# williamyang1991/VToonify

Hardware: NVIDIA H100
Metric: frames/sec at 576x1024 (higher is better)
Workload: dtype bf16x3 (fp32 operands split into bf16 hi+lo, 3 tensor-core products, fp32 accumulate)

## Files before the change

vtoonify_b200/csrc/conv_tc.cu:

```cuda
#include "tc_common.cuh"
#include <cuda_bf16.h>
#include <mutex>

using namespace vt_tc;

int vt_validate_conv_desc(const vt_conv_desc* d, const char* who);
extern int g_upfirdn_tiled;
extern int g_smalln_is;
extern int g_fir4;
extern int g_instnorm_chunks;
extern int g_rs_kernel;
int vt_conv_rs_takes(const vt_conv_desc* d);
int vt_conv_rs_run(const vt_conv_desc* d, void* stream);

namespace {

constexpr int TILE_W = 8, TILE_H = 16, TILE_M = 128;
constexpr int KCH = 32;
constexpr int MAX_SMEM = 227 * 1024;
constexpr int MAX_BLOCK_N = 128;
constexpr int MAX_ACC_COLS = 128;
constexpr int WIDE_N = 256;
constexpr int WIDE_REGS_XFORM = 88;
constexpr int WIDE_REGS_CONSUMER = 208;
constexpr int STATS_WARPS = 8;

struct TcArgs {
  CUtensorMap in_map[2][4];
  CUtensorMap w_map;
  int n_src, kchunks[2], coff[2];
  int n_steps;
  int8_t step_view[VT_MAX_TAPS], step_vx[VT_MAX_TAPS], step_vy[VT_MAX_TAPS];
  int16_t step_w[VT_MAX_TAPS];
  int step_aoff[VT_MAX_TAPS];
  int n_phase;
  int tgroup;
  int halo, halo_x0, halo_y0, halo_w;
  int n_hv, hv_view[4], hv_x0[4], hv_y0[4], hv_off[4], hv_bytes[4], a_rows;
  uint16_t step_sbo[VT_MAX_TAPS];
  int a_stages, b_stages, a_stage_bytes, b_stage_bytes, a_tx_bytes, b_tx_bytes;
  int block_n, n_tiles, tiles_x, tiles_y, B, total_tiles;
  int m_first;
  int Ho, Wo, Cout, wB, out_cpitch;
  const float* bias;
  const float* noise;
  const float* noise_w;
  const float* res;
  float* out;
  int64_t out_sb, out_sy, out_sx, phase_off[4];
  int64_t pix_sb, pix_sy, pix_sx, phase_pix[4];
  int act, round_tf32;
  float slope, gain, alpha, beta;
  const float* rgb_w; const float* rgb_bias; const float* rgb_skip; const float* rgb_skip_kernel; float* rgb_out;
  const float* slope_vec;
  const float* src_scale[2];
  const float* src_affine[2];
  int src_cn[2];
  int64_t sc_sb, sc_sy, sc_sx;
  int in_w, in_h;
  int mma_n;
  int m_major;
  float* stats_ws;
  float acc_scale;
};

constexpr int TC_THREADS = 384;
constexpr int XFORM_WARPS = 3;
constexpr int CONSUMERS = 2;
constexpr int RELEASE_ARRIVALS = CONSUMERS * 4;

enum TcOp : int {
  OP_TF32 = 0,
  OP_BF16 = 1,
  OP_F16 = 2,
  OP_BF16_NSTACK = 3,
};

template <int NW, bool F16>
__device__ __forceinline__ void wgmma_split(float* acc, uint64_t a, uint64_t b, uint32_t accumulate) {
  if constexpr (NW == 32) {
    if constexpr (F16) wgmma_f16_n32(acc, a, b, accumulate); else wgmma_bf16_n32(acc, a, b, accumulate);
  } else if constexpr (NW == 64) {
    if constexpr (F16) wgmma_f16_n64(acc, a, b, accumulate); else wgmma_bf16_n64(acc, a, b, accumulate);
  } else if constexpr (NW == 128) {
    if constexpr (F16) wgmma_f16_n128(acc, a, b, accumulate); else wgmma_bf16_n128(acc, a, b, accumulate);
  } else {
    static_assert(NW == WIDE_N && !F16, "the 256-wide MMA exists for the bf16 split only");
    wgmma_bf16_n256(acc, a, b, accumulate);
  }
}

template <int NW, int OP>
__device__ __forceinline__ void mma_step(float* acc, uint64_t adesc, uint64_t bdesc, uint32_t first) {
  if constexpr (OP == OP_TF32) {
    if constexpr (NW == 32) {
      wgmma_tf32_n32(acc, adesc, bdesc, first ^ 1u); wgmma_tf32_n32(acc, adesc + 2, bdesc + 2, 1);
      wgmma_tf32_n32(acc, adesc + 4, bdesc + 4, 1); wgmma_tf32_n32(acc, adesc + 6, bdesc + 6, 1);
    } else if constexpr (NW == 64) {
      wgmma_tf32_n64(acc, adesc, bdesc, first ^ 1u); wgmma_tf32_n64(acc, adesc + 2, bdesc + 2, 1);
      wgmma_tf32_n64(acc, adesc + 4, bdesc + 4, 1); wgmma_tf32_n64(acc, adesc + 6, bdesc + 6, 1);
    } else {
      wgmma_tf32_n128(acc, adesc, bdesc, first ^ 1u); wgmma_tf32_n128(acc, adesc + 2, bdesc + 2, 1);
      wgmma_tf32_n128(acc, adesc + 4, bdesc + 4, 1); wgmma_tf32_n128(acc, adesc + 6, bdesc + 6, 1);
    }
  } else {
    constexpr bool nstack = OP == OP_BF16_NSTACK;
    constexpr int ao[6] = {0, 2, 4, 6, 0, 2};
    constexpr int bo[6] = {0, 2, 0, 2, 4, 6};
#pragma unroll
    for (int i = 0; i < (nstack ? 4 : 6); ++i)
      wgmma_split<NW, OP == OP_F16>(acc, adesc + (uint64_t)ao[i], bdesc + (uint64_t)(nstack ? ao[i] : bo[i]), i == 0 ? (first ^ 1u) : 1u);
  }
}

template <int NW, int MT, int OP>
__global__ void __launch_bounds__(TC_THREADS, 1)
conv_tc_kernel(const __grid_constant__ TcArgs p) {
  constexpr bool WIDE = NW == WIDE_N;
  static_assert((MT * NW <= MAX_ACC_COLS || (WIDE && MT == 1 && OP == OP_BF16)) && (MT == 1 || MT == 2 || MT == 4),
                "accumulators of one work item exceed the register plan");
  static_assert(128 * WIDE_REGS_XFORM + 256 * WIDE_REGS_CONSUMER <= TC_THREADS * ((65536 / TC_THREADS) & ~7),
                "setmaxnreg plan exceeds the launch allocation");
  static_assert(OP != OP_BF16_NSTACK || NW == 64, "the N-stacked form is the Cout == 32 layer at MMA N = 64");
  constexpr bool SPLIT = OP != OP_TF32;
  extern __shared__ uint8_t smem_raw[];
  const uint32_t smem_base = (smem_u32(smem_raw) + 1023u) & ~1023u;
  const uint32_t a_base = smem_base;
  const uint32_t b_base = a_base + (uint32_t)p.a_stages * p.a_stage_bytes;
  const uint32_t bar_base = b_base + (uint32_t)p.b_stages * p.b_stage_bytes;
  auto a_full = [&](int i) { return bar_base + 8u * i; };
  auto a_empty = [&](int i) { return bar_base + 64u + 8u * i; };
  auto b_full = [&](int i) { return bar_base + 128u + 8u * i; };
  auto b_empty = [&](int i) { return bar_base + 192u + 8u * i; };
  auto a_ready = [&](int i) { return bar_base + 256u + 8u * i; };

  const int warp = threadIdx.x >> 5, lane = threadIdx.x & 31;
  const int wg = threadIdx.x >> 7;

  if (warp == 0 && lane == 0) {
    for (int s = 0; s < p.n_src; ++s)
      for (int v = 0; v < 4; ++v) tma_prefetch_desc(&p.in_map[s][v]);
    tma_prefetch_desc(&p.w_map);
  }
  if (warp == 1 && lane == 0) {
    for (int i = 0; i < p.a_stages; ++i) { mbar_init(a_full(i), 1); mbar_init(a_empty(i), RELEASE_ARRIVALS); mbar_init(a_ready(i), XFORM_WARPS); }
    for (int i = 0; i < p.b_stages; ++i) { mbar_init(b_full(i), 1); mbar_init(b_empty(i), RELEASE_ARRIVALS); }
    fence_barrier_init();
    fence_proxy_async_smem();
  }
  __syncthreads();

  const int m_tiles = p.total_tiles / p.n_tiles;
  const int tiles_per_img = p.tiles_y * p.tiles_x;
  constexpr int item_w = TILE_W * MT;

  if (wg == 0) {
    if constexpr (WIDE) asm volatile("setmaxnreg.dec.sync.aligned.u32 %0;" ::"n"(WIDE_REGS_XFORM));
    if (warp == 0) {
      int a_st = 0, b_st = 0;
      uint32_t a_par = 0, b_par = 0;
      for (int tile = blockIdx.x; tile < p.total_tiles; tile += gridDim.x) {
        const int n_tile = p.m_major ? tile % p.n_tiles : tile / m_tiles, m = p.m_first + (p.m_major ? tile / p.n_tiles : tile % m_tiles);
        const int b = m / tiles_per_img, rem = m % tiles_per_img;
        const int oy0 = (rem / p.tiles_x) * TILE_H, ox0 = (rem % p.tiles_x) * item_w;
        const int n0 = n_tile * p.block_n;
        const int wb = p.wB > 1 ? b : 0;
        for (int s = 0; s < p.n_src; ++s) {
          for (int kc = 0; kc < p.kchunks[s]; ++kc) {
            const int c0 = kc * KCH;
            if (p.halo) {
              mbar_wait(a_empty(a_st), a_par ^ 1);
              if (elect_one()) {
                const uint32_t st = a_base + a_st * p.a_stage_bytes;
                mbar_arrive_expect_tx(a_full(a_st), (uint32_t)p.a_tx_bytes);
                for (int v = 0; v < p.n_hv; ++v)
                  tma_load_4d(st + p.hv_off[v], &p.in_map[s][p.hv_view[v]], a_full(a_st), c0, ox0 + p.hv_x0[v], oy0 + p.hv_y0[v], b);
              }
              __syncwarp();
              if (++a_st == p.a_stages) { a_st = 0; a_par ^= 1; }
            }
            int gj = 0;
            for (int j = 0; j < p.n_steps; ++j) {
              if (!p.halo) {
                mbar_wait(a_empty(a_st), a_par ^ 1);
                if (elect_one()) {
                  mbar_arrive_expect_tx(a_full(a_st), (uint32_t)p.a_tx_bytes);
                  tma_load_4d(a_base + a_st * p.a_stage_bytes, &p.in_map[s][p.step_view[j]], a_full(a_st), c0, ox0 + p.step_vx[j],
                              oy0 + p.step_vy[j], b);
                }
                __syncwarp();
                if (++a_st == p.a_stages) { a_st = 0; a_par ^= 1; }
              }
              if (gj == 0) {
                mbar_wait(b_empty(b_st), b_par ^ 1);
                if (elect_one()) {
                  const int wc = SPLIT ? (p.coff[s] + c0) * 2 : p.coff[s] + c0;
                  mbar_arrive_expect_tx(b_full(b_st), (uint32_t)p.b_tx_bytes);
                  tma_load_4d(b_base + b_st * p.b_stage_bytes, &p.w_map, b_full(b_st), wc, OP == OP_BF16_NSTACK ? 0 : n0, p.step_w[j], wb);
                }
                __syncwarp();
                if (++b_st == p.b_stages) { b_st = 0; b_par ^= 1; }
              }
              if (++gj == p.tgroup) gj = 0;
            }
          }
        }
      }
    } else if constexpr (SPLIT) {
      const int t = (warp - 1) * 32 + lane;
      const int rows = p.a_rows;
      int a_st = 0;
      uint32_t a_par = 0;
      const int bw = p.halo ? p.halo_w : TILE_W;
      for (int tile = blockIdx.x; tile < p.total_tiles; tile += gridDim.x) {
        const int m = p.m_first + (p.m_major ? tile / p.n_tiles : tile % m_tiles);
        const int b = m / tiles_per_img, rem = m % tiles_per_img;
        const int oy0 = (rem / p.tiles_x) * TILE_H, ox0 = (rem % p.tiles_x) * item_w;
        for (int s = 0; s < p.n_src; ++s) {
          const float* sc = p.src_scale[s];
          const float* aff = p.src_affine[s];
          for (int kc = 0; kc < p.kchunks[s]; ++kc) {
            const float4* affp = aff ? reinterpret_cast<const float4*>(aff + ((int64_t)b * p.src_cn[s] + kc * KCH) * 2) : nullptr;
            const int loads = p.halo ? 1 : p.n_steps;
            for (int l = 0; l < loads; ++l) {
              mbar_wait(a_full(a_st), a_par);
              const uint32_t stage = a_base + a_st * p.a_stage_bytes;
              const int bx0 = ox0 + (p.halo ? p.halo_x0 : p.step_vx[l]), by0 = oy0 + (p.halo ? p.halo_y0 : p.step_vy[l]);
              for (int r = t; r < rows; r += 32 * XFORM_WARPS) {
                const uint32_t row = stage + (uint32_t)r * 128u;
                const uint32_t ph = (row >> 7) & 7u;
                float f[32];
#pragma unroll
                for (int j = 0; j < 8; ++j) {
                  float4 v;
                  asm volatile("ld.shared.v4.f32 {%0, %1, %2, %3}, [%4];" : "=f"(v.x), "=f"(v.y), "=f"(v.z), "=f"(v.w) : "r"(row + ((j ^ ph) << 4)));
                  f[4 * j] = v.x; f[4 * j + 1] = v.y; f[4 * j + 2] = v.z; f[4 * j + 3] = v.w;
                }
                if (sc || aff) {
                  const int ry = r / bw, rx = r - ry * bw;
                  const int ix = bx0 + rx, iy = by0 + ry;
                  const bool inb = ix >= 0 && ix < p.in_w && iy >= 0 && iy < p.in_h;
                  if (aff && inb) {
#pragma unroll
                    for (int j = 0; j < 16; ++j) {
                      const float4 q = __ldg(affp + j);
                      f[2 * j] = fmaf(f[2 * j], q.x, q.y);
                      f[2 * j + 1] = fmaf(f[2 * j + 1], q.z, q.w);
                    }
                  }
                  if (sc) {
                    const float mm = inb ? __ldg(sc + (int64_t)b * p.sc_sb + (int64_t)iy * p.sc_sy + (int64_t)ix * p.sc_sx) : 0.f;
#pragma unroll
                    for (int i = 0; i < 32; ++i) f[i] *= mm;
                  }
                }
                uint32_t hi[16], lo[16];
                if constexpr (OP == OP_F16) {
#pragma unroll
                  for (int i = 0; i < 16; ++i) split_f16x2(f[2 * i], f[2 * i + 1], hi[i], lo[i]);
                } else {
#pragma unroll
                  for (int i = 0; i < 16; ++i) {
                    const __nv_bfloat162 h2 = __floats2bfloat162_rn(f[2 * i], f[2 * i + 1]);
                    hi[i] = *reinterpret_cast<const uint32_t*>(&h2);
                    const float r0 = f[2 * i] - __uint_as_float(hi[i] << 16), r1 = f[2 * i + 1] - __uint_as_float(hi[i] & 0xffff0000u);
                    const __nv_bfloat162 l2 = __floats2bfloat162_rn(r0, r1);
                    lo[i] = *reinterpret_cast<const uint32_t*>(&l2);
                  }
                }
#pragma unroll
                for (int m4 = 0; m4 < 4; ++m4) {
                  asm volatile("st.shared.v4.b32 [%0], {%1, %2, %3, %4};" ::"r"(row + ((m4 ^ ph) << 4)), "r"(hi[4 * m4]), "r"(hi[4 * m4 + 1]), "r"(hi[4 * m4 + 2]), "r"(hi[4 * m4 + 3]) : "memory");
                  asm volatile("st.shared.v4.b32 [%0], {%1, %2, %3, %4};" ::"r"(row + (((m4 + 4) ^ ph) << 4)), "r"(lo[4 * m4]), "r"(lo[4 * m4 + 1]), "r"(lo[4 * m4 + 2]), "r"(lo[4 * m4 + 3]) : "memory");
                }
              }
              fence_proxy_async_smem();
              __syncwarp();
              if (lane == 0) mbar_arrive(a_ready(a_st));
              if (++a_st == p.a_stages) { a_st = 0; a_par ^= 1; }
            }
          }
        }
      }
    }
  } else {
    if constexpr (WIDE) asm volatile("setmaxnreg.inc.sync.aligned.u32 %0;" ::"n"(WIDE_REGS_CONSUMER));
    const int c = wg - 1;
    const int tw_ = (threadIdx.x & 127) >> 5;
    const bool leader = lane == 0;
    const int qd = lane & 3;
    float acc[MT][NW / 2];
#pragma unroll
    for (int g = 0; g < MT; ++g)
#pragma unroll
      for (int i = 0; i < NW / 2; ++i) acc[g][i] = 0.f;
    const float nw = (p.noise && p.noise_w) ? *p.noise_w : 0.f;
    int a_st = 0, b_st = 0;
    uint32_t a_par = 0, b_par = 0;
    const uint32_t tile_bytes_n = (uint32_t)p.mma_n * 128u;
    for (int tile = blockIdx.x; tile < p.total_tiles; tile += gridDim.x) {
      const int n_tile = p.m_major ? tile % p.n_tiles : tile / m_tiles, m = p.m_first + (p.m_major ? tile / p.n_tiles : tile % m_tiles);
      const int b = m / tiles_per_img, rem = m % tiles_per_img;
      const int oy0 = (rem / p.tiles_x) * TILE_H, ox0 = (rem % p.tiles_x) * item_w;
      const int n0 = n_tile * p.block_n;
      uint32_t first = 1;
      int rel_a = -1, rel_b = -1;
      for (int s = 0; s < p.n_src; ++s) {
        for (int kc = 0; kc < p.kchunks[s]; ++kc) {
          if (p.halo) mbar_wait(SPLIT ? a_ready(a_st) : a_full(a_st), a_par);
          int gj = 0;
          for (int j = 0; j < p.n_steps; ++j) {
            if (!p.halo) mbar_wait(SPLIT ? a_ready(a_st) : a_full(a_st), a_par);
            if (gj == 0) mbar_wait(b_full(b_st), b_par);
            uint32_t a_addr = a_base + a_st * p.a_stage_bytes;
            uint32_t sbo = 1024;
            if (p.halo) {
              a_addr += (uint32_t)p.step_aoff[j];
              sbo = (uint32_t)p.step_sbo[j];
            }
            a_addr += 8u * (uint32_t)c * sbo;
            const uint64_t bdesc = make_smem_desc_sw128(b_base + b_st * p.b_stage_bytes + (uint32_t)gj * tile_bytes_n, 1024);
            const bool last_of_group = (gj == p.tgroup - 1);
            wgmma_fence();
#pragma unroll
            for (int g = 0; g < MT; ++g) {
              const uint64_t adesc = make_smem_desc_sw128(a_addr + (uint32_t)(g * TILE_W * 128), sbo);
              mma_step<NW, OP>(acc[g], adesc, bdesc, first);
            }
            wgmma_commit();
            wgmma_wait<1>();
            if (leader) {
              if (rel_a >= 0) mbar_arrive(a_empty(rel_a));
              if (rel_b >= 0) mbar_arrive(b_empty(rel_b));
            }
            rel_a = (!p.halo || j == p.n_steps - 1) ? a_st : -1;
            rel_b = last_of_group ? b_st : -1;
            first = 0;
            if (last_of_group) { gj = 0; if (++b_st == p.b_stages) { b_st = 0; b_par ^= 1; } } else { ++gj; }
            if (!p.halo || j == p.n_steps - 1) { if (++a_st == p.a_stages) { a_st = 0; a_par ^= 1; } }
          }
        }
      }
      wgmma_wait<0>();
#pragma unroll
      for (int g = 0; g < MT; ++g) wgmma_pin<NW / 2>(acc[g]);
      if (leader) {
        if (rel_a >= 0) mbar_arrive(a_empty(rel_a));
        if (rel_b >= 0) mbar_arrive(b_empty(rel_b));
      }

      const int r0 = 64 * c + 16 * tw_ + (lane >> 2);
      const int ty = r0 / TILE_W, tx = r0 % TILE_W;
      const int ph0 = n0 / p.Cout, nb0 = n0 - ph0 * p.Cout;
      const int nchunks = p.block_n / 32;
#pragma unroll
      for (int g = 0; g < MT; ++g) {
        int oy[2], ox[2];
        bool in_img[2];
        int64_t off0[2], pix0[2];
        float rgb[2][3] = {{0.f, 0.f, 0.f}, {0.f, 0.f, 0.f}};
#pragma unroll
        for (int h = 0; h < 2; ++h) {
          oy[h] = oy0 + ty + h; ox[h] = ox0 + g * TILE_W + tx;
          in_img[h] = oy[h] < p.Ho && ox[h] < p.Wo;
          off0[h] = (int64_t)b * p.out_sb + (int64_t)oy[h] * p.out_sy + (int64_t)ox[h] * p.out_sx;
          pix0[h] = (int64_t)b * p.pix_sb + (int64_t)oy[h] * p.pix_sy + (int64_t)ox[h] * p.pix_sx;
        }
        int ph = ph0, nb = nb0 - 32;
#pragma unroll
        for (int j = 0; j < NW / 32; ++j) {
          if (j >= nchunks) break;
          nb += 32;
          if (nb >= p.Cout) { nb -= p.Cout; ++ph; }
          float nz[2];
#pragma unroll
          for (int h = 0; h < 2; ++h) nz[h] = (p.noise && in_img[h]) ? nw * __ldg(p.noise + p.phase_pix[ph] + pix0[h]) : 0.f;
          float v[2][4][2];
#pragma unroll
          for (int k = 0; k < 4; ++k)
#pragma unroll
            for (int h = 0; h < 2; ++h)
#pragma unroll
              for (int e = 0; e < 2; ++e) {
                const int i = 16 * j + 4 * k + 2 * h + e;
                float x = acc[g][i];
                if constexpr (OP == OP_BF16_NSTACK) x += acc[g][(i + 16) % (NW / 2)];
                v[h][k][e] = x * p.acc_scale;
              }
#pragma unroll
          for (int k = 0; k < 4; ++k) {
            const int ch = nb + 8 * k + 2 * qd;
            float2 bq = make_float2(0.f, 0.f), sq = make_float2(p.slope, p.slope);
            if (p.bias) bq = __ldg(reinterpret_cast<const float2*>(p.bias + ch));
            if (p.slope_vec) sq = __ldg(reinterpret_cast<const float2*>(p.slope_vec + ch));
#pragma unroll
            for (int h = 0; h < 2; ++h) {
              float v0 = v[h][k][0] + bq.x + nz[h], v1 = v[h][k][1] + bq.y + nz[h];
              if (p.act == VT_ACT_LRELU) {
                v0 = vt_lrelu(v0, sq.x) * p.gain; v1 = vt_lrelu(v1, sq.y) * p.gain;
              } else if (!WIDE && p.act == VT_ACT_RELU_TANH) {
                v0 = tanhf(fmaxf(v0, 0.f)); v1 = tanhf(fmaxf(v1, 0.f));
              }
              const int64_t off = p.phase_off[ph] + off0[h] + ch;
              if (p.res) {
                if (in_img[h]) {
                  const float2 rv = __ldg(reinterpret_cast<const float2*>(p.res + off));
                  v0 = v0 * p.alpha + p.beta * rv.x; v1 = v1 * p.alpha + p.beta * rv.y;
                }
              } else if (p.alpha != 1.f) {
                v0 *= p.alpha; v1 *= p.alpha;
              }
              if (p.round_tf32) { v0 = vt_round_tf32(v0); v1 = vt_round_tf32(v1); }
              if (!WIDE && p.rgb_w) {
                const float* w0 = p.rgb_w + ((int64_t)(p.wB > 1 ? b : 0) * 3) * p.Cout + ch;
#pragma unroll
                for (int cc = 0; cc < 3; ++cc) {
                  const float2 wv = __ldg(reinterpret_cast<const float2*>(w0 + cc * p.Cout));
                  rgb[h][cc] = fmaf(v1, wv.y, fmaf(v0, wv.x, rgb[h][cc]));
                }
              }
              if (in_img[h] && p.out) *reinterpret_cast<float2*>(p.out + off) = make_float2(v0, v1);
              v[h][k][0] = in_img[h] ? v0 : 0.f; v[h][k][1] = in_img[h] ? v1 : 0.f;
            }
          }
          if (p.stats_ws) {
            const int kchunk = ((rem * MT + g) * STATS_WARPS) + c * 4 + tw_;
            float2* wsp = reinterpret_cast<float2*>(p.stats_ws) + ((int64_t)kchunk * p.B + b) * p.Cout + nb + 2 * qd;
#pragma unroll
            for (int k = 0; k < 4; ++k)
#pragma unroll
              for (int e = 0; e < 2; ++e) {
                float ssum = v[0][k][e] + v[1][k][e];
                float ssq = fmaf(v[0][k][e], v[0][k][e], v[1][k][e] * v[1][k][e]);
#pragma unroll
                for (int o = 4; o < 32; o <<= 1) {
                  ssum += __shfl_xor_sync(0xffffffffu, ssum, o);
                  ssq += __shfl_xor_sync(0xffffffffu, ssq, o);
                }
                if (lane < 4) wsp[8 * k + e] = make_float2(ssum, ssq);
              }
          }
        }
        if (!WIDE && p.rgb_w) {
#pragma unroll
          for (int h = 0; h < 2; ++h)
#pragma unroll
            for (int cc = 0; cc < 3; ++cc) {
              rgb[h][cc] += __shfl_xor_sync(0xffffffffu, rgb[h][cc], 1);
              rgb[h][cc] += __shfl_xor_sync(0xffffffffu, rgb[h][cc], 2);
            }
#pragma unroll
          for (int h = 0; h < 2; ++h) {
            if (qd != 0 || !in_img[h]) continue;
            torgb_store(p.rgb_bias, p.rgb_skip, p.rgb_skip_kernel, p.rgb_out, rgb[h], b, oy[h], ox[h], p.Ho, p.Wo);
          }
        }
      }
    }
  }
}

struct TcKernel {
  int nw, mt, op;
  void (*fn)(TcArgs);
};
#define VT_TC_OPS(NW, MT) {NW, MT, OP_TF32, conv_tc_kernel<NW, MT, OP_TF32>}, {NW, MT, OP_BF16, conv_tc_kernel<NW, MT, OP_BF16>}, \
                          {NW, MT, OP_F16, conv_tc_kernel<NW, MT, OP_F16>}
const TcKernel kTcKernels[] = {
    VT_TC_OPS(128, 1), VT_TC_OPS(64, 1), VT_TC_OPS(64, 2), VT_TC_OPS(32, 1), VT_TC_OPS(32, 2), VT_TC_OPS(32, 4),
    {64, 1, OP_BF16_NSTACK, conv_tc_kernel<64, 1, OP_BF16_NSTACK>}, {64, 2, OP_BF16_NSTACK, conv_tc_kernel<64, 2, OP_BF16_NSTACK>},
    {WIDE_N, 1, OP_BF16, conv_tc_kernel<WIDE_N, 1, OP_BF16>},
};
#undef VT_TC_OPS

}

typedef CUresult (*PFN_encodeTiled)(CUtensorMap*, CUtensorMapDataType, cuuint32_t, void*, const cuuint64_t*,
                                    const cuuint64_t*, const cuuint32_t*, const cuuint32_t*, CUtensorMapInterleave,
                                    CUtensorMapSwizzle, CUtensorMapL2promotion, CUtensorMapFloatOOBfill);

static PFN_encodeTiled get_encode() {
  static PFN_encodeTiled fn = nullptr;
  static std::once_flag once;
  std::call_once(once, [] {
    void* f = nullptr;
    cudaDriverEntryPointQueryResult qres;
    if (cudaGetDriverEntryPoint("cuTensorMapEncodeTiled", &f, cudaEnableDefault, &qres) == cudaSuccess &&
        qres == cudaDriverEntryPointSuccess)
      fn = (PFN_encodeTiled)f;
  });
  return fn;
}

int vt_tc_make_map4(CUtensorMap* m, const void* base, const uint64_t dims[4], const uint64_t strides_b[3], const uint32_t box[4],
                    const char* what, bool bf16) {
  PFN_encodeTiled enc = get_encode();
  VT_CHECK(enc != nullptr, "conv_tc: cuTensorMapEncodeTiled not available from the driver");
  cuuint64_t gd[4] = {dims[0], dims[1], dims[2], dims[3]};
  cuuint64_t gs[3] = {strides_b[0], strides_b[1], strides_b[2]};
  cuuint32_t bx[4] = {box[0], box[1], box[2], box[3]};
  cuuint32_t es[4] = {1, 1, 1, 1};
  for (int i = 0; i < 4; ++i) VT_CHECK(gd[i] >= 1 && bx[i] >= 1 && bx[i] <= 256, "conv_tc: bad %s map dim %d (dim=%llu box=%u)", what, i, (unsigned long long)gd[i], bx[i]);
  for (int i = 0; i < 3; ++i) VT_CHECK(gs[i] % 16 == 0 && gs[i] > 0, "conv_tc: %s map stride %d (%llu B) not a positive multiple of 16", what, i, (unsigned long long)gs[i]);
  VT_CHECK(((uintptr_t)base & 15) == 0, "conv_tc: %s base pointer not 16-byte aligned", what);
  CUresult r = enc(m, bf16 ? CU_TENSOR_MAP_DATA_TYPE_BFLOAT16 : CU_TENSOR_MAP_DATA_TYPE_FLOAT32, 4, const_cast<void*>(base), gd, gs, bx, es,
                   CU_TENSOR_MAP_INTERLEAVE_NONE, CU_TENSOR_MAP_SWIZZLE_128B, CU_TENSOR_MAP_L2_PROMOTION_L2_256B,
                   CU_TENSOR_MAP_FLOAT_OOB_FILL_NONE);
  VT_CHECK(r == CUDA_SUCCESS, "conv_tc: cuTensorMapEncodeTiled(%s) failed with CUresult %d", what, (int)r);
  return 0;
}


namespace {
inline int make_map4(CUtensorMap* m, const void* base, const uint64_t dims[4], const uint64_t strides_b[3], const uint32_t box[4],
                     const char* what, bool bf16 = false) { return vt_tc_make_map4(m, base, dims, strides_b, box, what, bf16); }

int g_tc_mode = 1;
int g_tc_mt = 0;
int g_tc_transpose = 1;
int g_tc_tgroup = 0;
int g_tc_s2_halo = 0;
int g_tc_stage_policy = 1;
int g_tc_halo_pct = 60;
int g_tc_m_major = 1;
int g_tc_wide = 1;

int check_supported(const vt_conv_desc* d, bool set_err) {
#define VT_SUP(cond, ...) do { if (!(cond)) { if (set_err) vt_set_error(__VA_ARGS__); return 0; } } while (0)
  VT_SUP(d->Cout % 32 == 0, "conv_tc: Cout must be a multiple of 32 (got %d)", d->Cout);
  VT_SUP(d->out != nullptr || d->rgb_w != nullptr, "conv_tc: out may be NULL only with the fused ToRGB tail (image-only launch)");
  for (int s = 0; s < d->n_src; ++s) {
    VT_SUP(d->src_c[s] % KCH == 0, "conv_tc: src_c[%d]=%d must be a multiple of 32", s, d->src_c[s]);
    VT_SUP(d->src_cstride[s] % 4 == 0, "conv_tc: channel stride must be a multiple of 4");
  }
  VT_SUP(d->stride == 1 || d->stride == 2, "conv_tc: stride must be 1 or 2");
  VT_SUP(d->n_phase == 1 || (d->n_phase == 4 && d->stride == 1 && g_tc_mode != 0 && !d->res), "conv_tc: phases need stride 1, halo mode, no residual");
  for (int ph = 0; ph < d->n_phase; ++ph) VT_SUP(d->phase_off[ph] % 4 == 0, "conv_tc: phase offset must be a multiple of 4 floats");
  VT_SUP(d->out_sx % 4 == 0 && d->out_sy % 4 == 0 && d->out_sb % 4 == 0, "conv_tc: output strides must be multiples of 4 floats");
  VT_SUP(((uintptr_t)d->out & 15) == 0, "conv_tc: out not 16-byte aligned");
  VT_SUP(d->w_cstride % 4 == 0, "conv_tc: weight stride must be a multiple of 4");
  VT_SUP((!d->src_scale[0] && !d->src_scale[1] && !d->src_affine[0] && !d->src_affine[1]) || (d->weight_bf16x3 && d->stride == 1),
         "conv_tc: src_scale / src_affine need the bf16x3 mode and stride 1");
  for (int s = 0; s < 2; ++s) VT_SUP(!d->src_affine[s] || (((uintptr_t)d->src_affine[s] & 15) == 0), "conv_tc: src_affine not 16-byte aligned");
  VT_SUP(!d->bf16x3_nstack || (d->weight_bf16x3 && d->Cout == 32 && d->n_phase == 1 && d->split_fmt == 0), "conv_tc: the N-stacked bf16x3 form needs Cout == 32, one phase and the bf16 split");
  VT_SUP(d->split_fmt == 0 || d->split_fmt == 1, "conv_tc: split_fmt must be 0 (bf16) or 1 (fp16)");
  VT_SUP(!d->weight_bf16x3 || d->w_cstride % KCH == 0, "conv_tc: bf16x3 weights need a channel stride that is a multiple of 32");
  VT_SUP(!d->res || (((uintptr_t)d->res & 15) == 0), "conv_tc: res not 16-byte aligned");
  VT_SUP(!d->bias || (((uintptr_t)d->bias & 15) == 0), "conv_tc: bias not 16-byte aligned");
  VT_SUP(!d->slope_vec || (((uintptr_t)d->slope_vec & 15) == 0), "conv_tc: slope_vec not 16-byte aligned");
  VT_SUP(!d->rgb_w || (d->n_phase == 1 && d->Cout <= MAX_BLOCK_N && (d->Cout & (d->Cout - 1)) == 0 && (((uintptr_t)d->rgb_w & 15) == 0) &&
                       d->out_sx == d->Cout && d->out_sy == (int64_t)d->Wo * d->Cout && (!d->rgb_skip || (d->Ho % 2 == 0 && d->Wo % 2 == 0))),
         "conv_tc: fused ToRGB needs Cout a power of two <= 128, one phase, a dense output and even Ho/Wo for the skip");
  return 1;
#undef VT_SUP
}

}

extern "C" int vt_set_option(const char* key, int value) {
  if (key && strcmp(key, "tc_mode") == 0) { int old = g_tc_mode; g_tc_mode = value; return old; }
  if (key && strcmp(key, "tc_mt") == 0) { int old = g_tc_mt; g_tc_mt = value; return old; }
  if (key && strcmp(key, "tc_tgroup") == 0) { int old = g_tc_tgroup; g_tc_tgroup = value; return old; }
  if (key && strcmp(key, "tc_s2_halo") == 0) { int old = g_tc_s2_halo; g_tc_s2_halo = value; return old; }
  if (key && strcmp(key, "tc_stage_policy") == 0) { int old = g_tc_stage_policy; g_tc_stage_policy = value; return old; }
  if (key && strcmp(key, "tc_halo_pct") == 0) { int old = g_tc_halo_pct; g_tc_halo_pct = value; return old; }
  if (key && strcmp(key, "tc_m_major") == 0) { int old = g_tc_m_major; g_tc_m_major = value; return old; }
  if (key && strcmp(key, "tc_transpose") == 0) { int old = g_tc_transpose; g_tc_transpose = value; return old; }
  if (key && strcmp(key, "tc_wide") == 0) { int old = g_tc_wide; g_tc_wide = value; return old; }
  if (key && strcmp(key, "rs_kernel") == 0) { int old = g_rs_kernel; g_rs_kernel = value; return old; }
  if (key && strcmp(key, "instnorm_chunks") == 0) { int old = g_instnorm_chunks; g_instnorm_chunks = value; return old; }
  if (key && strcmp(key, "fir4") == 0) { int old = g_fir4; g_fir4 = value; return old; }
  if (key && strcmp(key, "smalln_is") == 0) { int old = g_smalln_is; g_smalln_is = value; return old; }
  if (key && strcmp(key, "upfirdn_tiled") == 0) { int old = g_upfirdn_tiled; g_upfirdn_tiled = value; return old; }
  return -1;
}

extern "C" int vt_conv2d_tc_supported(const vt_conv_desc* d) {
  if (!d || d->struct_size != (int)sizeof(vt_conv_desc)) return 0;
  return check_supported(d, false);
}

static int conv_tc_run(const vt_conv_desc* d, void* stream, int* chunks_out, int m_first = 0, bool allow_wide = true) {
  if (vt_validate_conv_desc(d, "conv2d_tc")) return 1;
  if (!check_supported(d, true)) return 1;

  static thread_local TcArgs a;
  memset(&a, 0, sizeof(a));

  bool T = false;
  if (g_tc_transpose && d->stride == 1 && !d->rgb_w) {
    const int64_t t0 = vt_cdiv(d->Wo, TILE_W) * vt_cdiv(d->Ho, TILE_H), t1 = vt_cdiv(d->Ho, TILE_W) * vt_cdiv(d->Wo, TILE_H);
    T = (g_tc_transpose == 2) || (t1 < t0);
  }
  const int gH = T ? d->W : d->H, gW = T ? d->H : d->W, gHo = T ? d->Wo : d->Ho, gWo = T ? d->Ho : d->Wo;
  const int64_t g_out_sy = T ? d->out_sx : d->out_sy, g_out_sx = T ? d->out_sy : d->out_sx;

  a.n_phase = d->n_phase;
  a.Ho = gHo; a.Wo = gWo; a.Cout = d->Cout; a.wB = d->wB; a.out_cpitch = d->out_cpitch;
  a.bias = d->bias; a.noise = d->noise; a.noise_w = d->noise_w; a.res = d->res;
  a.out_sb = d->out_sb; a.out_sy = g_out_sy; a.out_sx = g_out_sx;
  for (int ph = 0; ph < 4; ++ph) a.phase_off[ph] = d->phase_off[ph < d->n_phase ? ph : 0];
  if (d->noise) {
    VT_CHECK(d->out_sb % d->out_cpitch == 0 && d->out_sy % d->out_cpitch == 0 && d->out_sx % d->out_cpitch == 0,
             "conv_tc: output strides must be multiples of out_cpitch when noise is used");
    a.pix_sb = d->out_sb / d->out_cpitch; a.pix_sy = g_out_sy / d->out_cpitch; a.pix_sx = g_out_sx / d->out_cpitch;
    for (int ph = 0; ph < 4; ++ph) {
      VT_CHECK(a.phase_off[ph] % d->out_cpitch == 0, "conv_tc: phase offset must be a multiple of out_cpitch");
      a.phase_pix[ph] = a.phase_off[ph] / d->out_cpitch;
    }
  }
  a.out = d->out;
  a.slope_vec = d->slope_vec;
  a.rgb_w = d->rgb_w; a.rgb_bias = d->rgb_bias; a.rgb_skip = d->rgb_skip; a.rgb_skip_kernel = d->rgb_skip_kernel; a.rgb_out = d->rgb_out;
  a.act = d->act; a.round_tf32 = d->round_tf32; a.slope = d->slope; a.gain = d->gain; a.alpha = d->alpha; a.beta = d->beta;
  a.B = d->B;
  const bool split = d->weight_bf16x3 != nullptr;
  const bool nstack = split && d->bf16x3_nstack;
  const int op = !split ? OP_TF32 : nstack ? OP_BF16_NSTACK : d->split_fmt == 1 ? OP_F16 : OP_BF16;
  a.acc_scale = (split && d->acc_scale > 0.f) ? d->acc_scale : 1.f;
  a.src_scale[0] = d->src_scale[0]; a.src_scale[1] = d->src_scale[1];
  a.src_affine[0] = d->src_affine[0]; a.src_affine[1] = d->src_affine[1];
  a.src_cn[0] = d->src_c[0]; a.src_cn[1] = d->n_src > 1 ? d->src_c[1] : 0;
  a.in_w = gW; a.in_h = gH;
  a.sc_sb = (int64_t)d->H * d->W; a.sc_sy = T ? 1 : d->W; a.sc_sx = T ? d->W : 1;

  a.n_src = d->n_src;
  int coff = 0;
  for (int s = 0; s < d->n_src; ++s) { a.kchunks[s] = d->src_c[s] / KCH; a.coff[s] = coff; coff += d->src_c[s]; }
  a.n_steps = d->taps;
  int dxmin = 1 << 30, dxmax = -(1 << 30), dymin = 1 << 30, dymax = -(1 << 30);
  for (int t = 0; t < d->taps; ++t) {
    const int tdx = T ? d->tap_dy[t] : d->tap_dx[t], tdy = T ? d->tap_dx[t] : d->tap_dy[t];
    int view = 0, vx = tdx, vy = tdy;
    if (d->stride == 2) {
      const int px = tdx & 1, py = tdy & 1;
      view = py * 2 + px;
      vx = (tdx - px) / 2;
      vy = (tdy - py) / 2;
    }
    VT_CHECK(vx >= -100 && vx <= 100 && vy >= -100 && vy <= 100, "conv_tc: tap offset out of range");
    a.step_view[t] = (int8_t)view; a.step_vx[t] = (int8_t)vx; a.step_vy[t] = (int8_t)vy;
    a.step_w[t] = (int16_t)d->tap_w[t];
    dxmin = vx < dxmin ? vx : dxmin; dxmax = vx > dxmax ? vx : dxmax;
    dymin = vy < dymin ? vy : dymin; dymax = vy > dymax ? vy : dymax;
  }

  const int n_eff = d->n_phase * d->Cout;
  int bn_narrow = MAX_BLOCK_N;
  while (bn_narrow > 32 && (n_eff % bn_narrow) != 0) bn_narrow /= 2;
  VT_CHECK(n_eff % bn_narrow == 0, "conv_tc: no N tile for N=%d", n_eff);
  const bool wide = allow_wide && (g_tc_wide == 2 || (g_tc_wide == 1 && d->stride == 1)) && op == OP_BF16 && n_eff % WIDE_N == 0 &&
                    !d->rgb_w && d->act != VT_ACT_RELU_TANH;
  const int bn = wide ? WIDE_N : bn_narrow;
  const int bnm = nstack ? 2 * bn : bn;
  const bool can_halo = (g_tc_mode != 0) && (d->taps > 1 || (bn <= 64 && d->stride == 1)) && (d->stride == 1 || g_tc_mode != 3);
  int mt = 1;
  if (can_halo && g_tc_mt != 1) {
    int want = (g_tc_mt > 0) ? g_tc_mt : (bn >= 128 ? 1 : (bn >= 64 ? 2 : 4));
    while (want > 1 && (want * bnm > MAX_ACC_COLS || gWo <= TILE_W * (want / 2))) want /= 2;
    mt = want;
  }
  const int fixed = 1024  + 1024 ;
  int smem_bytes = 0;
  int tgroup = 1;
  if (g_tc_tgroup != 1) {
    for (int tg = d->taps; tg >= 2; --tg) {
      if (d->taps % tg != 0 || tg * bnm * 128 > (g_tc_tgroup > 1 ? g_tc_tgroup : 36) * 1024) continue;
      bool ok = true;
      for (int t = 0; t < d->taps && ok; ++t)
        if (t % tg != 0 && d->tap_w[t] != d->tap_w[t - 1] + 1) ok = false;
      if (ok) { tgroup = tg; break; }
    }
  }
  a.tgroup = tgroup;
  int vx0[4], vx1[4], vy0[4], vy1[4];
  bool vused[4] = {false, false, false, false};
  for (int t = 0; t < d->taps; ++t) {
    const int v = a.step_view[t], vx = a.step_vx[t], vy = a.step_vy[t];
    if (!vused[v]) { vused[v] = true; vx0[v] = vx1[v] = vx; vy0[v] = vy1[v] = vy; }
    vx0[v] = vx < vx0[v] ? vx : vx0[v]; vx1[v] = vx > vx1[v] ? vx : vx1[v];
    vy0[v] = vy < vy0[v] ? vy : vy0[v]; vy1[v] = vy > vy1[v] ? vy : vy1[v];
  }
  int hv_w[4] = {0, 0, 0, 0}, hv_h[4] = {0, 0, 0, 0};
  for (;; mt /= 2) {
    int halo_bytes = 0, tx_bytes = 0;
    bool fits = true;
    a.n_hv = 0;
    for (int v = 0; v < 4; ++v) {
      if (!vused[v]) continue;
      const int w = TILE_W * mt + (vx1[v] - vx0[v]), h = TILE_H + (vy1[v] - vy0[v]);
      fits = fits && w <= 256 && h <= 256;
      const int i = a.n_hv++;
      a.hv_view[i] = v; a.hv_x0[i] = vx0[v]; a.hv_y0[i] = vy0[v]; a.hv_off[i] = halo_bytes; a.hv_bytes[i] = w * h * 128;
      hv_w[v] = w; hv_h[v] = h;
      tx_bytes += w * h * 128;
      halo_bytes = (int)(vt_cdiv(halo_bytes + w * h * 128, 1024) * 1024);
    }
    const int64_t tap_bytes = (int64_t)d->taps * TILE_M * 128;
    const bool pays = (d->stride == 2 && g_tc_s2_halo) ? (tx_bytes * 10 <= tap_bytes * 6) : ((int64_t)tx_bytes * 100 <= tap_bytes * g_tc_halo_pct);
    a.halo = can_halo && fits && halo_bytes <= 96 * 1024 && (mt > 1 || pays) &&
             2 * halo_bytes + 2 * bnm * 128 * tgroup + fixed <= MAX_SMEM;
    if (!a.halo && mt > 1) continue;
    a.halo_x0 = a.hv_x0[0]; a.halo_y0 = a.hv_y0[0]; a.halo_w = hv_w[a.hv_view[0]];
    a.a_tx_bytes = a.halo ? tx_bytes : TILE_M * 128;
    a.a_rows = a.halo ? (a.hv_off[a.n_hv - 1] + a.hv_bytes[a.n_hv - 1]) / 128 : TILE_M;
    a.a_stage_bytes = a.halo ? halo_bytes : TILE_M * 128;
    a.b_stage_bytes = bnm * 128 * tgroup;
    a.a_stages = a.halo ? 3 : 4;
    a.b_stages = tgroup > 1 ? 4 : 6;
    const int b_floor = (g_tc_stage_policy == 1 && a.halo && a.a_stage_bytes >= 40 * 1024 && tgroup == 1) ? 5 : 3;
    while (a.a_stages * a.a_stage_bytes + a.b_stages * a.b_stage_bytes + fixed > MAX_SMEM) {
      if (a.b_stages > b_floor) --a.b_stages;
      else if (a.a_stages > 2) --a.a_stages;
      else if (a.b_stages > 2) --a.b_stages;
      else break;
    }
    if (b_floor > 3)
      while (a.b_stages < 8 && a.a_stages * a.a_stage_bytes + (a.b_stages + 1) * a.b_stage_bytes + fixed <= MAX_SMEM) ++a.b_stages;
    smem_bytes = a.a_stages * a.a_stage_bytes + a.b_stages * a.b_stage_bytes + fixed;
    if (smem_bytes <= MAX_SMEM || mt == 1) break;
  }
  if (wide && !(smem_bytes <= MAX_SMEM && a.a_stages >= 2 && a.b_stages >= 3)) return conv_tc_run(d, stream, chunks_out, m_first, false);
  a.b_tx_bytes = bnm * 128 * tgroup;
  VT_CHECK(smem_bytes <= MAX_SMEM && a.a_stages >= 2 && a.b_stages >= 2 && a.a_stages <= 8 && a.b_stages <= 8,
           "conv_tc: shared memory plan does not fit (%d B, mt=%d, bn=%d)", smem_bytes, mt, bn);
  for (int t = 0; t < d->taps; ++t) {
    const int v = a.step_view[t];
    int i = 0;
    while (i < a.n_hv - 1 && a.hv_view[i] != v) ++i;
    a.step_aoff[t] = a.hv_off[i] + ((a.step_vy[t] - vy0[v]) * hv_w[v] + (a.step_vx[t] - vx0[v])) * 128;
    a.step_sbo[t] = (uint16_t)(hv_w[v] * 128);
  }
  a.block_n = bn;
  a.mma_n = bnm;
  a.n_tiles = n_eff / bn;
  VT_CHECK(!d->rgb_w || a.n_tiles == 1, "conv_tc: fused ToRGB needs one N tile (Cout = %d)", d->Cout);
  a.tiles_x = (int)vt_cdiv(gWo, TILE_W * mt);
  a.tiles_y = (int)vt_cdiv(gHo, TILE_H);
  const int64_t m_total = (int64_t)a.B * a.tiles_x * a.tiles_y;
  VT_CHECK(m_first < m_total, "conv_tc: first pixel tile %d out of range", m_first);
  const int64_t total = (int64_t)a.n_tiles * (m_total - m_first);
  VT_CHECK(total < (1LL << 31), "conv_tc: too many tiles");
  a.total_tiles = (int)total;
  a.m_first = m_first;
  a.m_major = g_tc_m_major ? 1 : 0;
  {
    const int64_t chunks = (int64_t)a.tiles_x * a.tiles_y * mt * STATS_WARPS;
    if (chunks_out) {
      VT_CHECK(d->n_phase == 1 && !d->rgb_w && chunks < (1 << 24), "conv_tc: output statistics need one phase and no fused ToRGB");
      *chunks_out = (int)chunks;
      return 0;
    }
    if (d->stats_ws) {
      VT_CHECK(d->n_phase == 1 && !d->rgb_w, "conv_tc: output statistics need one phase and no fused ToRGB");
      VT_CHECK(d->stats_ws_floats >= chunks * d->B * d->Cout * 2, "conv_tc: stats_ws too small (%lld floats, need %lld)",
               (long long)d->stats_ws_floats, (long long)(chunks * d->B * d->Cout * 2));
      VT_CHECK(((uintptr_t)d->stats_ws & 7) == 0, "conv_tc: stats_ws not 8-byte aligned");
      a.stats_ws = d->stats_ws;
    }
  }

  for (int s = 0; s < d->n_src; ++s) {
    const uint64_t cs = (uint64_t)d->src_cstride[s];
    if (d->stride == 1) {
      const uint64_t real_sx = cs * 4, real_sy = (uint64_t)d->W * cs * 4;
      const uint64_t dims[4] = {cs, (uint64_t)gW, (uint64_t)gH, (uint64_t)d->B};
      const uint64_t str[3] = {T ? real_sy : real_sx, T ? real_sx : real_sy, (uint64_t)d->H * d->W * cs * 4};
      const uint32_t box[4] = {KCH, (uint32_t)(a.halo ? hv_w[0] : TILE_W), (uint32_t)(a.halo ? hv_h[0] : TILE_H), 1};
      if (make_map4(&a.in_map[s][0], d->src[s], dims, str, box, "input")) return 1;
      for (int v = 1; v < 4; ++v) a.in_map[s][v] = a.in_map[s][0];
    } else {
      bool have0 = false;
      for (int py = 0; py < 2; ++py)
        for (int px = 0; px < 2; ++px) {
          const int vw = (d->W - px + 1) / 2, vh = (d->H - py + 1) / 2;
          CUtensorMap* mp = &a.in_map[s][py * 2 + px];
          if (vw < 1 || vh < 1) { if (have0) *mp = a.in_map[s][0]; continue; }
          const uint64_t dims[4] = {cs, (uint64_t)vw, (uint64_t)vh, (uint64_t)d->B};
          const uint64_t str[3] = {2 * cs * 4, 2 * (uint64_t)d->W * cs * 4, (uint64_t)d->H * d->W * cs * 4};
          const int v = py * 2 + px;
          const uint32_t box[4] = {KCH, (uint32_t)((a.halo && vused[v]) ? hv_w[v] : TILE_W), (uint32_t)((a.halo && vused[v]) ? hv_h[v] : TILE_H), 1};
          if (make_map4(mp, d->src[s] + ((int64_t)py * d->W + px) * cs, dims, str, box, "input(parity)")) return 1;
          have0 = true;
        }
    }
  }
  {
    const uint64_t wc = (uint64_t)d->w_cstride;
    const uint64_t dims[4] = {wc, (uint64_t)n_eff, (uint64_t)d->w_taps, (uint64_t)d->wB};
    const uint64_t str[3] = {wc * 4, (uint64_t)n_eff * wc * 4, (uint64_t)d->w_taps * n_eff * wc * 4};
    if (split) {
      VT_CHECK(((uintptr_t)d->weight_bf16x3 & 15) == 0, "conv_tc: weight_bf16x3 not 16-byte aligned");
      const uint64_t rows = (uint64_t)n_eff * (nstack ? 2 : 1);
      const uint64_t dims2[4] = {2 * wc, rows, (uint64_t)d->w_taps, (uint64_t)d->wB};
      const uint64_t str2[3] = {wc * 4, rows * wc * 4, (uint64_t)d->w_taps * rows * wc * 4};
      const uint32_t box[4] = {2 * KCH, (uint32_t)bnm, (uint32_t)a.tgroup, 1};
      if (make_map4(&a.w_map, d->weight_bf16x3, dims2, str2, box, "weight(bf16x3)", true)) return 1;
    } else {
      const uint32_t box[4] = {KCH, (uint32_t)bn, (uint32_t)a.tgroup, 1};
      if (make_map4(&a.w_map, d->weight, dims, str, box, "weight")) return 1;
    }
  }
  static std::once_flag attr_once;
  static cudaError_t attr_err = cudaSuccess;
  std::call_once(attr_once, [] {
    for (const TcKernel& k : kTcKernels)
      if (attr_err == cudaSuccess) attr_err = cudaFuncSetAttribute(k.fn, cudaFuncAttributeMaxDynamicSharedMemorySize, MAX_SMEM);
  });
  VT_CHECK(attr_err == cudaSuccess, "conv_tc: cudaFuncSetAttribute failed: %s", cudaGetErrorString(attr_err));
  const TcKernel* kern = nullptr;
  for (const TcKernel& k : kTcKernels)
    if (k.nw == bnm && k.mt == mt && k.op == op) kern = &k;
  if (!kern) return vt_set_error("conv_tc: no kernel for MMA N = %d, %d M tiles, operand mode %d", bnm, mt, op);
  int grid = vt_num_sms();
  int m_split = 0;
  if (wide && g_tc_wide == 1 && a.total_tiles >= grid && a.total_tiles % grid != 0)
    m_split = (a.total_tiles / grid) * grid / a.n_tiles;
  if (m_split > 0) a.total_tiles = m_split * a.n_tiles;
  if (grid > a.total_tiles) grid = a.total_tiles;
  kern->fn<<<grid, TC_THREADS, smem_bytes, (cudaStream_t)stream>>>(a);
  VT_LAUNCH_CHECK();
  return m_split > 0 ? conv_tc_run(d, stream, nullptr, m_split, false) : 0;
}

extern "C" int vt_conv2d_tc_tf32(const vt_conv_desc* d, void* stream) { return conv_tc_run(d, stream, nullptr); }

static bool rs_shape(const vt_conv_desc* d) {
  if (d->n_src != 1 || d->stride != 1 || d->taps != 9 || d->n_phase != 1 || d->res || d->slope_vec || !d->weight_bf16x3) return false;
  if (d->src_scale[0] || d->src_affine[0] || d->alpha != 1.f) return false;
  if ((d->Cout != 32 && d->Cout != 64) || (d->src_c[0] != 32 && d->src_c[0] != 64)) return false;
  return d->act == VT_ACT_NONE || d->act == VT_ACT_LRELU;
}

extern "C" int vt_conv2d_rs_supported(const vt_conv_desc* d) {
  if (!d || d->struct_size != (int)sizeof(vt_conv_desc)) return 0;
  return rs_shape(d) && check_supported(d, false);
}

extern "C" int vt_conv2d_rs(const vt_conv_desc* d, float acc_scale, void* stream) {
  VT_CHECK(d && d->struct_size == (int)sizeof(vt_conv_desc) && rs_shape(d), "conv2d_rs: not a row-strip layer (3x3, stride 1, Cin/Cout in {32, 64})");
  vt_conv_desc c = *d;
  if (acc_scale > 0.f) c.acc_scale = acc_scale;
  if (g_rs_kernel && vt_conv_rs_takes(&c)) return vt_conv_rs_run(&c, stream);
  return conv_tc_run(&c, stream, nullptr);
}

extern "C" int vt_conv2d_tc_stats_chunks(const vt_conv_desc* d) {
  int chunks = 0;
  if (conv_tc_run(d, nullptr, &chunks)) return -1;
  return chunks;
}
```

Before: 37.02.

## Add ping-pong consumer warpgroup schedule for 128x128 bf16-split conv tiles

Adds a ping-pong variant of the tensor-core conv kernel in which the two consumer warpgroups take alternate tiles. Each warpgroup computes the full 128-row tile, and a pair of turn barriers orders their MMA phases so one group's epilogue overlaps the other's MMAs. Registers are rebalanced with setmaxnreg to hold the doubled accumulators, and the epilogue's noise and residual loads are prefetched. It is selected only for large tile counts with 128-wide bf16 split items and no rgb or tanh epilogue. The cost is more register pressure and extra barrier traffic.

```diff
diff --git a/vtoonify_b200/csrc/conv_tc.cu b/vtoonify_b200/csrc/conv_tc.cu
--- a/vtoonify_b200/csrc/conv_tc.cu
+++ b/vtoonify_b200/csrc/conv_tc.cu
@@ -113,12 +113,15 @@
   }
 }
 
-template <int NW, int MT, int OP>
-__global__ void __launch_bounds__(TC_THREADS, 1)
-conv_tc_kernel(const __grid_constant__ TcArgs p) {
+template <int NW, int MT, int OP, bool PP>
+__device__ __forceinline__ void conv_tc_body(const TcArgs& p) {
   constexpr bool WIDE = NW == WIDE_N;
+  constexpr bool REALLOC = WIDE || PP;
+  constexpr int HALVES = PP ? 2 : 1;
   static_assert((MT * NW <= MAX_ACC_COLS || (WIDE && MT == 1 && OP == OP_BF16)) && (MT == 1 || MT == 2 || MT == 4),
                 "accumulators of one work item exceed the register plan");
+  static_assert(!PP || (NW == MAX_BLOCK_N && MT == 1 && OP == OP_BF16), "the ping-pong item is the 128 x 128 bf16-split item");
+  constexpr int RELEASES = PP ? 4 : RELEASE_ARRIVALS;
   static_assert(128 * WIDE_REGS_XFORM + 256 * WIDE_REGS_CONSUMER <= TC_THREADS * ((65536 / TC_THREADS) & ~7),
                 "setmaxnreg plan exceeds the launch allocation");
   static_assert(OP != OP_BF16_NSTACK || NW == 64, "the N-stacked form is the Cout == 32 layer at MMA N = 64");
@@ -133,6 +136,7 @@
   auto b_full = [&](int i) { return bar_base + 128u + 8u * i; };
   auto b_empty = [&](int i) { return bar_base + 192u + 8u * i; };
   auto a_ready = [&](int i) { return bar_base + 256u + 8u * i; };
+  auto turn = [&](int c) { return bar_base + 320u + 8u * c; };
 
   const int warp = threadIdx.x >> 5, lane = threadIdx.x & 31;
   const int wg = threadIdx.x >> 7;
@@ -143,8 +147,9 @@
     tma_prefetch_desc(&p.w_map);
   }
   if (warp == 1 && lane == 0) {
-    for (int i = 0; i < p.a_stages; ++i) { mbar_init(a_full(i), 1); mbar_init(a_empty(i), RELEASE_ARRIVALS); mbar_init(a_ready(i), XFORM_WARPS); }
-    for (int i = 0; i < p.b_stages; ++i) { mbar_init(b_full(i), 1); mbar_init(b_empty(i), RELEASE_ARRIVALS); }
+    for (int i = 0; i < p.a_stages; ++i) { mbar_init(a_full(i), 1); mbar_init(a_empty(i), RELEASES); mbar_init(a_ready(i), XFORM_WARPS); }
+    for (int i = 0; i < p.b_stages; ++i) { mbar_init(b_full(i), 1); mbar_init(b_empty(i), RELEASES); }
+    if constexpr (PP) { mbar_init(turn(0), 4); mbar_init(turn(1), 4); }
     fence_barrier_init();
     fence_proxy_async_smem();
   }
@@ -155,7 +160,7 @@
   constexpr int item_w = TILE_W * MT;
 
   if (wg == 0) {
-    if constexpr (WIDE) asm volatile("setmaxnreg.dec.sync.aligned.u32 %0;" ::"n"(WIDE_REGS_XFORM));
+    if constexpr (REALLOC) asm volatile("setmaxnreg.dec.sync.aligned.u32 %0;" ::"n"(WIDE_REGS_XFORM));
     if (warp == 0) {
       int a_st = 0, b_st = 0;
       uint32_t a_par = 0, b_par = 0;
@@ -284,25 +289,59 @@
       }
     }
   } else {
-    if constexpr (WIDE) asm volatile("setmaxnreg.inc.sync.aligned.u32 %0;" ::"n"(WIDE_REGS_CONSUMER));
+    if constexpr (REALLOC) asm volatile("setmaxnreg.inc.sync.aligned.u32 %0;" ::"n"(WIDE_REGS_CONSUMER));
     const int c = wg - 1;
     const int tw_ = (threadIdx.x & 127) >> 5;
     const bool leader = lane == 0;
     const int qd = lane & 3;
-    float acc[MT][NW / 2];
-#pragma unroll
-    for (int g = 0; g < MT; ++g)
+    float acc[MT * HALVES][NW / 2];
+#pragma unroll
+    for (int g = 0; g < MT * HALVES; ++g)
 #pragma unroll
       for (int i = 0; i < NW / 2; ++i) acc[g][i] = 0.f;
     const float nw = (p.noise && p.noise_w) ? *p.noise_w : 0.f;
     int a_st = 0, b_st = 0;
     uint32_t a_par = 0, b_par = 0;
     const uint32_t tile_bytes_n = (uint32_t)p.mma_n * 128u;
-    for (int tile = blockIdx.x; tile < p.total_tiles; tile += gridDim.x) {
+    int a_item = 0, b_item = 0;
+    uint32_t t_par = 0;
+    if constexpr (PP) {
+      for (int s = 0; s < p.n_src; ++s) {
+        a_item += p.halo ? p.kchunks[s] : p.kchunks[s] * p.n_steps;
+        b_item += p.kchunks[s] * (p.n_steps / p.tgroup);
+      }
+    }
+    for (int tile = blockIdx.x, item = 0; tile < p.total_tiles; tile += gridDim.x, ++item) {
       const int n_tile = p.m_major ? tile % p.n_tiles : tile / m_tiles, m = p.m_first + (p.m_major ? tile / p.n_tiles : tile % m_tiles);
       const int b = m / tiles_per_img, rem = m % tiles_per_img;
       const int oy0 = (rem / p.tiles_x) * TILE_H, ox0 = (rem % p.tiles_x) * item_w;
       const int n0 = n_tile * p.block_n;
+      if constexpr (PP) {
+        if ((item & 1) != c) {
+          for (a_st += a_item; a_st >= p.a_stages; a_st -= p.a_stages) a_par ^= 1;
+          for (b_st += b_item; b_st >= p.b_stages; b_st -= p.b_stages) b_par ^= 1;
+          continue;
+        }
+        const int ph_first = n0 / p.Cout, ph_last = (n0 + p.block_n - 1) / p.Cout;
+#pragma unroll
+        for (int hh = 0; hh < HALVES; ++hh)
+#pragma unroll
+          for (int h = 0; h < 2; ++h) {
+            const int r = 64 * hh + 16 * tw_ + (lane >> 2);
+            const int oy = oy0 + r / TILE_W + h, ox = ox0 + r % TILE_W;
+            if (oy >= p.Ho || ox >= p.Wo) continue;
+            if (p.noise) {
+              const int64_t pix = (int64_t)b * p.pix_sb + (int64_t)oy * p.pix_sy + (int64_t)ox * p.pix_sx;
+              for (int ph = ph_first; ph <= ph_last; ++ph) asm volatile("prefetch.global.L1 [%0];" ::"l"(p.noise + p.phase_pix[ph] + pix));
+            }
+            if (p.res) {
+              const int64_t off = p.phase_off[ph_first] + (int64_t)b * p.out_sb + (int64_t)oy * p.out_sy + (int64_t)ox * p.out_sx +
+                                  (n0 - ph_first * p.Cout) + 32 * qd;
+              asm volatile("prefetch.global.L2 [%0];" ::"l"(p.res + off));
+            }
+          }
+        if (item > 0) { mbar_wait(turn(c), t_par); t_par ^= 1; }
+      }
       uint32_t first = 1;
       int rel_a = -1, rel_b = -1;
       for (int s = 0; s < p.n_src; ++s) {
@@ -318,15 +357,17 @@
               a_addr += (uint32_t)p.step_aoff[j];
               sbo = (uint32_t)p.step_sbo[j];
             }
-            a_addr += 8u * (uint32_t)c * sbo;
+            if constexpr (!PP) a_addr += 8u * (uint32_t)c * sbo;
             const uint64_t bdesc = make_smem_desc_sw128(b_base + b_st * p.b_stage_bytes + (uint32_t)gj * tile_bytes_n, 1024);
             const bool last_of_group = (gj == p.tgroup - 1);
             wgmma_fence();
 #pragma unroll
-            for (int g = 0; g < MT; ++g) {
-              const uint64_t adesc = make_smem_desc_sw128(a_addr + (uint32_t)(g * TILE_W * 128), sbo);
-              mma_step<NW, OP>(acc[g], adesc, bdesc, first);
-            }
+            for (int g = 0; g < MT; ++g)
+#pragma unroll
+              for (int hh = 0; hh < HALVES; ++hh) {
+                const uint64_t adesc = make_smem_desc_sw128(a_addr + 8u * (uint32_t)hh * sbo + (uint32_t)(g * TILE_W * 128), sbo);
+                mma_step<NW, OP>(acc[g * HALVES + hh], adesc, bdesc, first);
+              }
             wgmma_commit();
             wgmma_wait<1>();
             if (leader) {
@@ -341,20 +382,24 @@
           }
         }
       }
+      if constexpr (PP) {
+        if (leader) mbar_arrive(turn(c ^ 1));
+      }
       wgmma_wait<0>();
 #pragma unroll
-      for (int g = 0; g < MT; ++g) wgmma_pin<NW / 2>(acc[g]);
+      for (int g = 0; g < MT * HALVES; ++g) wgmma_pin<NW / 2>(acc[g]);
       if (leader) {
         if (rel_a >= 0) mbar_arrive(a_empty(rel_a));
         if (rel_b >= 0) mbar_arrive(b_empty(rel_b));
       }
 
-      const int r0 = 64 * c + 16 * tw_ + (lane >> 2);
-      const int ty = r0 / TILE_W, tx = r0 % TILE_W;
       const int ph0 = n0 / p.Cout, nb0 = n0 - ph0 * p.Cout;
       const int nchunks = p.block_n / 32;
 #pragma unroll
-      for (int g = 0; g < MT; ++g) {
+      for (int gh = 0; gh < MT * HALVES; ++gh) {
+        const int g = gh / HALVES, half = PP ? gh % HALVES : c;
+        const int r0 = 64 * half + 16 * tw_ + (lane >> 2);
+        const int ty = r0 / TILE_W, tx = r0 % TILE_W;
         int oy[2], ox[2];
         bool in_img[2];
         int64_t off0[2], pix0[2];
@@ -383,8 +428,8 @@
 #pragma unroll
               for (int e = 0; e < 2; ++e) {
                 const int i = 16 * j + 4 * k + 2 * h + e;
-                float x = acc[g][i];
-                if constexpr (OP == OP_BF16_NSTACK) x += acc[g][(i + 16) % (NW / 2)];
+                float x = acc[gh][i];
+                if constexpr (OP == OP_BF16_NSTACK) x += acc[gh][(i + 16) % (NW / 2)];
                 v[h][k][e] = x * p.acc_scale;
               }
 #pragma unroll
@@ -398,7 +443,7 @@
               float v0 = v[h][k][0] + bq.x + nz[h], v1 = v[h][k][1] + bq.y + nz[h];
               if (p.act == VT_ACT_LRELU) {
                 v0 = vt_lrelu(v0, sq.x) * p.gain; v1 = vt_lrelu(v1, sq.y) * p.gain;
-              } else if (!WIDE && p.act == VT_ACT_RELU_TANH) {
+              } else if (!REALLOC && p.act == VT_ACT_RELU_TANH) {
                 v0 = tanhf(fmaxf(v0, 0.f)); v1 = tanhf(fmaxf(v1, 0.f));
               }
               const int64_t off = p.phase_off[ph] + off0[h] + ch;
@@ -411,7 +456,7 @@
                 v0 *= p.alpha; v1 *= p.alpha;
               }
               if (p.round_tf32) { v0 = vt_round_tf32(v0); v1 = vt_round_tf32(v1); }
-              if (!WIDE && p.rgb_w) {
+              if (!REALLOC && p.rgb_w) {
                 const float* w0 = p.rgb_w + ((int64_t)(p.wB > 1 ? b : 0) * 3) * p.Cout + ch;
 #pragma unroll
                 for (int cc = 0; cc < 3; ++cc) {
@@ -424,7 +469,7 @@
             }
           }
           if (p.stats_ws) {
-            const int kchunk = ((rem * MT + g) * STATS_WARPS) + c * 4 + tw_;
+            const int kchunk = ((rem * MT + g) * STATS_WARPS) + half * 4 + tw_;
             float2* wsp = reinterpret_cast<float2*>(p.stats_ws) + ((int64_t)kchunk * p.B + b) * p.Cout + nb + 2 * qd;
 #pragma unroll
             for (int k = 0; k < 4; ++k)
@@ -441,7 +486,7 @@
               }
           }
         }
-        if (!WIDE && p.rgb_w) {
+        if (!REALLOC && p.rgb_w) {
 #pragma unroll
           for (int h = 0; h < 2; ++h)
 #pragma unroll
@@ -460,16 +505,26 @@
   }
 }
 
+template <int NW, int MT, int OP>
+__global__ void __launch_bounds__(TC_THREADS, 1)
+conv_tc_kernel(const __grid_constant__ TcArgs p) { conv_tc_body<NW, MT, OP, false>(p); }
+
+template <int NW, int MT, int OP>
+__global__ void __launch_bounds__(TC_THREADS, 1)
+conv_tc_pingpong_kernel(const __grid_constant__ TcArgs p) { conv_tc_body<NW, MT, OP, true>(p); }
+
 struct TcKernel {
   int nw, mt, op;
+  bool pp;
   void (*fn)(TcArgs);
 };
-#define VT_TC_OPS(NW, MT) {NW, MT, OP_TF32, conv_tc_kernel<NW, MT, OP_TF32>}, {NW, MT, OP_BF16, conv_tc_kernel<NW, MT, OP_BF16>}, \
-                          {NW, MT, OP_F16, conv_tc_kernel<NW, MT, OP_F16>}
+#define VT_TC_OPS(NW, MT) {NW, MT, OP_TF32, false, conv_tc_kernel<NW, MT, OP_TF32>}, {NW, MT, OP_BF16, false, conv_tc_kernel<NW, MT, OP_BF16>}, \
+                          {NW, MT, OP_F16, false, conv_tc_kernel<NW, MT, OP_F16>}
 const TcKernel kTcKernels[] = {
     VT_TC_OPS(128, 1), VT_TC_OPS(64, 1), VT_TC_OPS(64, 2), VT_TC_OPS(32, 1), VT_TC_OPS(32, 2), VT_TC_OPS(32, 4),
-    {64, 1, OP_BF16_NSTACK, conv_tc_kernel<64, 1, OP_BF16_NSTACK>}, {64, 2, OP_BF16_NSTACK, conv_tc_kernel<64, 2, OP_BF16_NSTACK>},
-    {WIDE_N, 1, OP_BF16, conv_tc_kernel<WIDE_N, 1, OP_BF16>},
+    {64, 1, OP_BF16_NSTACK, false, conv_tc_kernel<64, 1, OP_BF16_NSTACK>}, {64, 2, OP_BF16_NSTACK, false, conv_tc_kernel<64, 2, OP_BF16_NSTACK>},
+    {WIDE_N, 1, OP_BF16, false, conv_tc_kernel<WIDE_N, 1, OP_BF16>},
+    {MAX_BLOCK_N, 1, OP_BF16, true, conv_tc_pingpong_kernel<MAX_BLOCK_N, 1, OP_BF16>},
 };
 #undef VT_TC_OPS
 
@@ -524,6 +579,7 @@
 int g_tc_halo_pct = 60;
 int g_tc_m_major = 1;
 int g_tc_wide = 1;
+int g_tc_pingpong = 1;
 
 int check_supported(const vt_conv_desc* d, bool set_err) {
 #define VT_SUP(cond, ...) do { if (!(cond)) { if (set_err) vt_set_error(__VA_ARGS__); return 0; } } while (0)
@@ -567,6 +623,7 @@
   if (key && strcmp(key, "tc_m_major") == 0) { int old = g_tc_m_major; g_tc_m_major = value; return old; }
   if (key && strcmp(key, "tc_transpose") == 0) { int old = g_tc_transpose; g_tc_transpose = value; return old; }
   if (key && strcmp(key, "tc_wide") == 0) { int old = g_tc_wide; g_tc_wide = value; return old; }
+  if (key && strcmp(key, "tc_pingpong") == 0) { int old = g_tc_pingpong; g_tc_pingpong = value; return old; }
   if (key && strcmp(key, "rs_kernel") == 0) { int old = g_rs_kernel; g_rs_kernel = value; return old; }
   if (key && strcmp(key, "instnorm_chunks") == 0) { int old = g_instnorm_chunks; g_instnorm_chunks = value; return old; }
   if (key && strcmp(key, "fir4") == 0) { int old = g_fir4; g_fir4 = value; return old; }
@@ -808,9 +865,11 @@
       if (attr_err == cudaSuccess) attr_err = cudaFuncSetAttribute(k.fn, cudaFuncAttributeMaxDynamicSharedMemorySize, MAX_SMEM);
   });
   VT_CHECK(attr_err == cudaSuccess, "conv_tc: cudaFuncSetAttribute failed: %s", cudaGetErrorString(attr_err));
+  const bool pingpong = (g_tc_pingpong == 2 || (g_tc_pingpong == 1 && a.total_tiles >= 3 * vt_num_sms())) && op == OP_BF16 &&
+                        bnm == MAX_BLOCK_N && mt == 1 && !d->rgb_w && d->act != VT_ACT_RELU_TANH;
   const TcKernel* kern = nullptr;
   for (const TcKernel& k : kTcKernels)
-    if (k.nw == bnm && k.mt == mt && k.op == op) kern = &k;
+    if (k.nw == bnm && k.mt == mt && k.op == op && k.pp == pingpong) kern = &k;
   if (!kern) return vt_set_error("conv_tc: no kernel for MMA N = %d, %d M tiles, operand mode %d", bnm, mt, op);
   int grid = vt_num_sms();
   int m_split = 0;
```

New measurement: 38.25, median of 6. +3.3%, better.
